# vbronetskyi/nclt-slam-project

Measured on AMD Instinct MI355X. Metric: relocalization frames/sec @640x480, 10k-landmark DB; Hamming-match HBM GB/s, higher is better.
Workload: dtype u8; 1 GPU; 640x480 BGR frames, 10000-record landmark DB (640000 descriptors, rows=fixed64), global relocalization tick per frame: ORB(500) + whole-DB mutual Hamming scan + top-25 PnP-RANSAC(200); frames resident in HBM, every frame's 96-byte result record written to pinned host memory by the tick's last kernel; distinct_frames=32, preroll_steps=20, streams=4, records=10000, descriptors=640000, parallelism=frames sharded across ranks, database replicated, no collective

## Files before the change

### include/reloc.h

```cpp
#ifndef RELOC_H
#define RELOC_H

#include <stdint.h>

#ifdef __cplusplus
extern "C" {
#endif

#define RELOC_OK            0
#define RELOC_E_ARG        (-1)
#define RELOC_E_NODEVICE   (-2)
#define RELOC_E_HIP        (-3)
#define RELOC_E_CAPACITY   (-4)
#define RELOC_E_STATE      (-5)

#define RELOC_ORDER_BGR 0
#define RELOC_ORDER_RGB 1

#define RELOC_OUT_PUBLISHED        0
#define RELOC_OUT_NO_FEATURES      1
#define RELOC_OUT_NO_CANDIDATES    2
#define RELOC_OUT_NO_PNP_ACCEPT    3
#define RELOC_OUT_CONSISTENCY_FAIL 4

// ... 12 lines not shown
    double heading_tol_deg;
    double reproj_max_px;
    double ransac_reproj_px;
    double ransac_confidence;
    double consistency_m;
    double global_reproj_max_px;
    double accum_min_dist_m;
    double accum_depth_min_m;
    double accum_depth_max_m;
    int32_t gray_coeff_bits;
    int32_t reserved0;
} reloc_params;

const char *reloc_last_error(void);
int  reloc_device_count(void);
reloc_ctx *reloc_create(int device, int max_w, int max_h, int max_feat);
void reloc_destroy(reloc_ctx *ctx);
int  reloc_set_stream(reloc_ctx *ctx, void *hip_stream);
int  reloc_sync(reloc_ctx *ctx);
void *reloc_dev_alloc(reloc_ctx *ctx, int64_t bytes);
int  reloc_dev_free(reloc_ctx *ctx, void *p);
int  reloc_h2d(reloc_ctx *ctx, void *dst_dev, const void *src_host, int64_t bytes);
int  reloc_d2d(reloc_ctx *ctx, void *dst_dev, const void *src_dev, int64_t bytes);
void *reloc_host_alloc(int64_t bytes);
int  reloc_host_free(void *p);
void *reloc_get_stream(reloc_ctx *ctx);
int  reloc_d2h(reloc_ctx *ctx, void *dst_host, const void *src_dev, int64_t bytes);
int  reloc_timer_begin(reloc_ctx *ctx);
int  reloc_timer_end(reloc_ctx *ctx, float *ms);
#define RELOC_PROF_DB_SCAN  0
#define RELOC_PROF_MATRIX   1
#define RELOC_PROF_ORB      2
#define RELOC_PROF_PNP      3
#define RELOC_PROF_STEREO   4
#define RELOC_PROF_STEREO_DENSE 5
#define RELOC_PROF_N        6
int  reloc_profile_enable(reloc_ctx *ctx, int on);
int  reloc_profile_get(reloc_ctx *ctx, int which, float *total_ms, int32_t *launches);

int  reloc_get_params(reloc_ctx *ctx, reloc_params *out);
int  reloc_set_params(reloc_ctx *ctx, const reloc_params *p);

int reloc_gray_u8(reloc_ctx *ctx, const uint8_t *img, int w, int h, int stride, int order,
                  uint8_t *gray);
int reloc_orb_detect_compute(reloc_ctx *ctx, const uint8_t *gray, int w, int h, int stride,
                             int nfeatures, float *xy, float *size, float *angle, float *response,
                             int32_t *octave, uint8_t *desc, int32_t *n_out);
int reloc_orb_frame_dev(reloc_ctx *ctx, const uint8_t *img_dev, int w, int h, int stride, int order,
                        int nfeatures);
const uint8_t *reloc_frame_desc_dev(reloc_ctx *ctx);
const float   *reloc_frame_xy_dev(reloc_ctx *ctx);
const int32_t *reloc_frame_count_dev(reloc_ctx *ctx);
int reloc_frame_debug_plane(reloc_ctx *ctx, int what, int level, uint8_t *out, int32_t *w, int32_t *h);

int reloc_set_orb_mask(reloc_ctx *ctx, const uint8_t *mask, int w, int h, int stride);
int reloc_get_orb_mask(reloc_ctx *ctx, int32_t *w, int32_t *h);
int reloc_orb_detect_compute_masked(reloc_ctx *ctx, const uint8_t *gray, int w, int h, int stride, const uint8_t *mask,
                                    int mask_stride, int nfeatures, float *xy, float *size, float *angle,
                                    float *response, int32_t *octave, uint8_t *desc, int32_t *n_out);
int reloc_orb_mask_level(reloc_ctx *ctx, int level, uint8_t *out, int32_t *w, int32_t *h);

int reloc_set_orb_params(reloc_ctx *ctx, int nlevels, double scale_factor, int fast_threshold, int score_type);
int reloc_get_orb_params(reloc_ctx *ctx, int32_t *nlevels, double *scale_factor, int32_t *fast_threshold, int32_t *score_type);
int reloc_orb_detect_compute_params(reloc_ctx *ctx, const uint8_t *gray, int w, int h, int stride, const uint8_t *mask,
                                    int mask_stride, int nfeatures, int nlevels, double scale_factor, int fast_threshold,
                                    int score_type, float *xy, float *size, float *angle, float *response,
                                    int32_t *octave, uint8_t *desc, int32_t *n_out);

int reloc_record_frame(reloc_ctx *ctx, const uint8_t *img, const uint16_t *depth_mm, int w, int h, int order,
                       int nfeatures, float *xy, uint8_t *desc, float *pts3d, int32_t *kp_index,
                       int32_t *n_out, int32_t *n_kp);

int reloc_depth_points(reloc_ctx *ctx, const void *depth, int is_f32, int w, int h, int step, const double K4[4],
                       float zmin, float zmax, float *points, int32_t *n_out);

int reloc_match_mutual(reloc_ctx *ctx, const uint8_t *q, int nq, const uint8_t *t, int nt,
                       int32_t *qidx, int32_t *tidx, int32_t *dist, int32_t *n_out);
int reloc_match_knn2(reloc_ctx *ctx, const uint8_t *q, int nq, const uint8_t *t, int nt,
                     int32_t *idx, int32_t *dist);
int reloc_match_ratio(reloc_ctx *ctx, const uint8_t *q, int nq, const uint8_t *t, int nt, double ratio,
                      int32_t *qidx, int32_t *tidx, int32_t *dist, int32_t *n_out);
#define RELOC_MATCH_CROSS 0
#define RELOC_MATCH_RATIO 1
int reloc_set_match_policy(reloc_ctx *ctx, int policy, double ratio);
int reloc_get_match_policy(reloc_ctx *ctx, int32_t *policy, double *ratio);
int reloc_db_upload(reloc_ctx *ctx, const uint8_t *desc, const float *pts3d, const int64_t *offsets,
                    const double *poses, int64_t n_records);
int64_t reloc_db_records(reloc_ctx *ctx);
int64_t reloc_db_rows(reloc_ctx *ctx);
int reloc_db_reserve(reloc_ctx *ctx, int64_t cap_records, int64_t cap_rows);
int reloc_db_append(reloc_ctx *ctx, const uint8_t *desc, const float *pts3d, const float *kp2d, int n,
                    const double pose[7], const double index_xy[2]);
int reloc_db_select(reloc_ctx *ctx, int slot);
int reloc_db_share(reloc_ctx *dst, reloc_ctx *src);
int reloc_db_fetch(reloc_ctx *ctx, int64_t record, uint8_t *desc, float *pts3d, float *kp2d, double pose[7],
                   double index_xyh[4], int32_t *n);
int reloc_db_match_counts(reloc_ctx *ctx, const uint8_t *cur, int n_cur, int32_t *counts);
int reloc_db_match_counts_dev(reloc_ctx *ctx, const uint8_t *cur_dev, const int32_t *n_cur_dev,
                              int n_cur_max, int32_t *counts_dev);
int reloc_db_ratio_counts(reloc_ctx *ctx, const uint8_t *cur, int n_cur, double ratio, int32_t *counts);
int reloc_hamming_matrix(reloc_ctx *ctx, const uint8_t *a, int64_t na, const uint8_t *b, int64_t nb,
                         uint16_t *out);
int reloc_hamming_matrix_dev(reloc_ctx *ctx, const uint8_t *a_dev, int64_t na, const uint8_t *b_dev,
                             int64_t nb, uint16_t *out_dev);

int reloc_pnp_score(reloc_ctx *ctx, const float *obj, const float *img, int m, const double *Rt, int H,
// ... 154 lines not shown
```

### nclt-slam-project_amd/_native.py

```python
from __future__ import annotations

import ctypes as C
import os

import numpy as np

_HERE = os.path.dirname(os.path.abspath(__file__))
LIB_PATH = (os.environ.get("RELOC_LIB") if os.environ.get("RELOC_DEV") == "1" else None) or os.path.join(_HERE, "csrc", "libreloc_hip.so")

c_ctx = C.c_void_p
i32, i64, u64, f32, f64 = C.c_int32, C.c_int64, C.c_uint64, C.c_float, C.c_double


class RelocError(RuntimeError):
    """Raised for every failure of the native library (the cv2 shim re-raises it as cv2.error)."""


class P:

    @classmethod
    def from_param(cls, a):
        if isinstance(a, np.ndarray):
            if not a.flags.c_contiguous:
                raise RelocError(f"a pointer argument must be a C-contiguous array, got strides {a.strides} for shape {a.shape}")
            return C.c_void_p(a.ctypes.data)
        if isinstance(a, (i32, i64, u64, f32, f64)):
            return C.byref(a)
        return C.c_void_p.from_param(a)


def outs(*types):
    return tuple(t() for t in types)


SIGNATURES = {
    "reloc_last_error": (C.c_char_p, []),
    "reloc_device_count": (C.c_int, []),
    "reloc_create": (c_ctx, [C.c_int, C.c_int, C.c_int, C.c_int]),
    "reloc_destroy": (None, [c_ctx]),
    "reloc_set_stream": (C.c_int, [c_ctx, P]),
    "reloc_sync": (C.c_int, [c_ctx]),
    "reloc_dev_alloc": (C.c_void_p, [c_ctx, i64]),
    "reloc_dev_free": (C.c_int, [c_ctx, P]),
    "reloc_h2d": (C.c_int, [c_ctx, P, P, i64]),
    "reloc_d2h": (C.c_int, [c_ctx, P, P, i64]),
    "reloc_timer_begin": (C.c_int, [c_ctx]),
    "reloc_timer_end": (C.c_int, [c_ctx, P]),
    "reloc_profile_enable": (C.c_int, [c_ctx, C.c_int]),
    "reloc_profile_get": (C.c_int, [c_ctx, C.c_int, P, P]),
    "reloc_gray_u8": (C.c_int, [c_ctx, P, C.c_int, C.c_int, C.c_int, C.c_int, P]),
    "reloc_orb_detect_compute": (C.c_int, [c_ctx, P, C.c_int, C.c_int, C.c_int, C.c_int, P, P, P, P, P, P, P]),
    "reloc_orb_frame_dev": (C.c_int, [c_ctx, P, C.c_int, C.c_int, C.c_int, C.c_int, C.c_int]),
    "reloc_frame_desc_dev": (C.c_void_p, [c_ctx]),
    "reloc_frame_xy_dev": (C.c_void_p, [c_ctx]),
    "reloc_frame_count_dev": (C.c_void_p, [c_ctx]),
    "reloc_frame_debug_plane": (C.c_int, [c_ctx, C.c_int, C.c_int, P, P, P]),
    "reloc_set_orb_mask": (C.c_int, [c_ctx, P, C.c_int, C.c_int, C.c_int]),
    "reloc_get_orb_mask": (C.c_int, [c_ctx, P, P]),
    "reloc_orb_detect_compute_masked": (C.c_int, [c_ctx, P, C.c_int, C.c_int, C.c_int, P, C.c_int, C.c_int, P, P, P, P, P, P, P]),
    "reloc_orb_mask_level": (C.c_int, [c_ctx, C.c_int, P, P, P]),
    "reloc_set_orb_params": (C.c_int, [c_ctx, C.c_int, f64, C.c_int, C.c_int]),
    "reloc_get_orb_params": (C.c_int, [c_ctx, P, P, P, P]),
    "reloc_orb_detect_compute_params": (C.c_int, [c_ctx, P, C.c_int, C.c_int, C.c_int, P, C.c_int, C.c_int, C.c_int, f64, C.c_int,
                                                  C.c_int, P, P, P, P, P, P, P]),
    "reloc_record_frame": (C.c_int, [c_ctx, P, P, C.c_int, C.c_int, C.c_int, C.c_int, P, P, P, P, P, P]),
    "reloc_depth_points": (C.c_int, [c_ctx, P, C.c_int, C.c_int, C.c_int, C.c_int, P, f32, f32, P, P]),
    "reloc_db_ratio_counts": (C.c_int, [c_ctx, P, C.c_int, f64, P]),
    "reloc_match_mutual": (C.c_int, [c_ctx, P, C.c_int, P, C.c_int, P, P, P, P]),
    "reloc_match_knn2": (C.c_int, [c_ctx, P, C.c_int, P, C.c_int, P, P]),
    "reloc_match_ratio": (C.c_int, [c_ctx, P, C.c_int, P, C.c_int, f64, P, P, P, P]),
    "reloc_set_match_policy": (C.c_int, [c_ctx, C.c_int, f64]),
    "reloc_get_match_policy": (C.c_int, [c_ctx, P, P]),
    "reloc_db_upload": (C.c_int, [c_ctx, P, P, P, P, i64]),
    "reloc_db_records": (i64, [c_ctx]),
    "reloc_db_rows": (i64, [c_ctx]),
    "reloc_db_counts_dev": (C.c_void_p, [c_ctx]),
    "reloc_db_match_counts": (C.c_int, [c_ctx, P, C.c_int, P]),
    "reloc_db_match_counts_dev": (C.c_int, [c_ctx, P, P, C.c_int, P]),
    "reloc_hamming_matrix": (C.c_int, [c_ctx, P, i64, P, i64, P]),
    "reloc_hamming_matrix_dev": (C.c_int, [c_ctx, P, i64, P, i64, P]),
    "reloc_pnp_score": (C.c_int, [c_ctx, P, P, C.c_int, P, C.c_int, P, f32, P, P]),
    "reloc_pnp_ransac": (C.c_int, [c_ctx, P, P, C.c_int, P, C.c_int, f32, f64, u64, P, P, P, P, P]),
    "reloc_pnp_debug_hypotheses": (C.c_int, [c_ctx, C.c_int, C.c_int, P, P, P]),
    "reloc_set_camera": (C.c_int, [c_ctx, P, P, P]),
    "reloc_set_distortion": (C.c_int, [c_ctx, P, C.c_int]),
    "reloc_get_distortion": (C.c_int, [c_ctx, P]),
    "reloc_undistort_points": (C.c_int, [c_ctx, P, C.c_int, P, P, P]),
    "reloc_pnp_score_dist": (C.c_int, [c_ctx, P, P, C.c_int, P, C.c_int, P, P, f32, P, P]),
    "reloc_pnp_ransac_dist": (C.c_int, [c_ctx, P, P, C.c_int, P, P, C.c_int, f32, f64, u64, P, P, P, P, P]),
    "reloc_set_clahe": (C.c_int, [c_ctx, f64, C.c_int, C.c_int]),
    "reloc_get_clahe": (C.c_int, [c_ctx, P, P, P]),
    "reloc_clahe_u8": (C.c_int, [c_ctx, P, C.c_int, C.c_int, C.c_int, f64, C.c_int, C.c_int, P]),
    "reloc_set_rectify_map": (C.c_int, [c_ctx, P, P, C.c_int, C.c_int]),
    "reloc_get_rectify_map": (C.c_int, [c_ctx, P, P]),
    "reloc_remap_u8": (C.c_int, [c_ctx, P, C.c_int, C.c_int, C.c_int, C.c_int, P, P, C.c_int, C.c_int, C.c_int, C.c_int, P]),
    "reloc_remap_u16": (C.c_int, [c_ctx, P, C.c_int, C.c_int, C.c_int, P, C.c_int, C.c_int, C.c_int, P]),
    "reloc_convert_maps": (C.c_int, [c_ctx, P, P, C.c_int, C.c_int, C.c_int, P, P]),
    "reloc_resize_u8": (C.c_int, [c_ctx, P, C.c_int, C.c_int, C.c_int, C.c_int, P, C.c_int, C.c_int, f64, f64, C.c_int]),
    "reloc_resize_u16": (C.c_int, [c_ctx, P, C.c_int, C.c_int, C.c_int, P, C.c_int, C.c_int, f64, f64]),
    "reloc_set_resize": (C.c_int, [c_ctx, C.c_int, C.c_int, C.c_int, C.c_int]),
    "reloc_get_resize": (C.c_int, [c_ctx, P, P, P, P]),
    "reloc_bayer_u8": (C.c_int, [c_ctx, P, C.c_int, C.c_int, C.c_int, C.c_int, P]),
    "reloc_set_bayer": (C.c_int, [c_ctx, C.c_int]),
    "reloc_get_bayer": (C.c_int, [c_ctx, P]),
    "reloc_cvt_gray_u8": (C.c_int, [c_ctx, P, C.c_int, C.c_int, C.c_int, C.c_int, P]),
    "reloc_yuv422_bgr_u8": (C.c_int, [c_ctx, P, C.c_int, C.c_int, C.c_int, C.c_int, C.c_int, P]),
    "reloc_set_pixel_format": (C.c_int, [c_ctx, C.c_int]),
    "reloc_get_pixel_format": (C.c_int, [c_ctx, P]),
    "reloc_set_stereo": (C.c_int, [c_ctx, f64, C.c_int, C.c_int, C.c_int, C.c_int]),
# ... 167 lines not shown
```

### nclt-slam-project_amd/csrc/reloc_orb.hip

```cpp
#include <math.h>

#include "../../include/reloc_orb_pattern.h"
#include "reloc_internal.h"
#include "reloc_pixels.h"

static_assert(HARRIS_CHUNK == 1024, "k_harris reads one dword per thread");

__constant__ signed char c_pattern[RELOC_ORB_NTESTS * 4];
__constant__ int c_umax[16] = {15, 15, 15, 15, 14, 14, 14, 13, 13, 12, 11, 10, 9, 8, 6, 3};
__constant__ signed char c_ring_dx[16] = {0, 1, 2, 3, 3, 3, 2, 1, 0, -1, -2, -3, -3, -3, -2, -1};
__constant__ signed char c_ring_dy[16] = {3, 3, 2, 1, 0, -1, -2, -3, -3, -3, -2, -1, 0, 1, 2, 3};

__device__ __forceinline__ int find_level(const int *base, int id)
{
    int l = 0;
#pragma unroll
    for (int k = 1; k < NLEV; ++k) l += id >= base[k];
    return l;
}


struct OrbBatch { OrbFrame f[RELOC_BATCH_MAX]; };

__device__ __forceinline__ void pyr_tab_index(const OrbTable *__restrict__ tab, const PyrTile &T, const int (&tbase)[NLEV + 1], int i,
// ... 308 lines not shown
        constexpr u32 sel_o = (u32)(o + 1) | 0x0C00u | (u32)(o + 3) << 16 | 0x0C000000u;
        const u32 ve = __builtin_amdgcn_perm(w[DY + 3][q + 1], w[DY + 3][q], sel_e);
        const u32 vo = __builtin_amdgcn_perm(w[DY + 3][q + 1], w[DY + 3][q], sel_o);
        tb[0] = ve + nb[0]; tb[1] = vo + nb[1];
        td[0] = nd[0] - ve; td[1] = nd[1] - vo;
    }
    template <int K>
    __device__ __forceinline__ void ring(u32 (&tb)[2], u32 (&td)[2]) const
    {
        constexpr int dx[16] = {0, 1, 2, 3, 3, 3, 2, 1, 0, -1, -2, -3, -3, -3, -2, -1};
        constexpr int dy[16] = {3, 3, 2, 1, 0, -1, -2, -3, -3, -3, -2, -1, 0, 1, 2, 3};
        flags<dx[K], dy[K]>(tb, td);
    }
    __device__ __forceinline__ bool candidate() const
    {
        u32 b0[2], d0[2], b4[2], d4[2], b8[2], d8[2], b12[2], d12[2];
        ring<0>(b0, d0); ring<4>(b4, d4); ring<8>(b8, d8); ring<12>(b12, d12);
        u32 any = 0;
#pragma unroll
        for (int j = 0; j < 2; ++j) {
            any |= (b0[j] & b4[j]) | (b8[j] & b12[j]) | ((b0[j] | b4[j]) & (b8[j] | b12[j]));
            any |= (d0[j] & d4[j]) | (d8[j] & d12[j]) | ((d0[j] | d4[j]) & (d8[j] | d12[j]));
        }
        return (any & 0x80008000u) != 0;
    }
    template <int K>
    __device__ __forceinline__ void shift_in(u32 (&mb)[2], u32 (&md)[2]) const
    {
        u32 tb[2], td[2];
        ring<K>(tb, td);
#pragma unroll
        for (int j = 0; j < 2; ++j) {
            mb[j] = (tb[j] & 0x80008000u) | ((mb[j] >> 1) & 0x7FFF7FFFu);
            md[j] = (td[j] & 0x80008000u) | ((md[j] >> 1) & 0x7FFF7FFFu);
        }
        if constexpr (K < 15) shift_in<K + 1>(mb, md);
    }
    __device__ __forceinline__ void masks(u32 (&mb)[2], u32 (&md)[2]) const
    {
        mb[0] = mb[1] = md[0] = md[1] = 0;
        shift_in<0>(mb, md);
    }
};

constexpr int FT_P = FT / 4 + 3;
static_assert(FT == 32, "fast_nms_tile maps 256 lanes to 32 rows x 8 dwords");
template <bool MASKED, int THR>
__device__ __forceinline__ void fast_nms_tile(const OrbTable *__restrict__ tab, const uint8_t *__restrict__ pyr,
                                              uint8_t *__restrict__ nms, int32_t *__restrict__ hist, int bid,
                                              const uint8_t *__restrict__ mask)
{
    __shared__ u32 s_img4[(FT + 8) * FT_P];
    __shared__ u32 s_sc4[(FT + 2) * (FT + 4) / 4];
    __shared__ unsigned short s_corner[(FT + 2) * (FT + 2)];
    __shared__ int s_nc;
    __shared__ int s_hist[256];
    const uint8_t *const s_img = reinterpret_cast<const uint8_t *>(s_img4);
    uint8_t *const s_sc = reinterpret_cast<uint8_t *>(s_sc4);
    const int l = find_level(tab->fast_tile_base, bid);
    const OrbLevel L = tab->lev[l];
    const int tile = bid - tab->fast_tile_base[l];
    const int tx = L.stride / FT;
    const int x0 = (tile % tx) * FT, y0 = (tile / tx) * FT;
    const int tid = threadIdx.x;
    const int e = RELOC_ORB_EDGE;
    const int thr = THR ? THR : tab->fast_thr;
    uint8_t *out = nms + L.off;
    const bool live = L.quota > 0 && x0 + FT > e && x0 < L.w - e && y0 + FT > e && y0 < L.h - e;
    if (!live) {
        const int y = y0 + tid / 8, x = x0 + (tid % 8) * 4;
        if (y < L.h) *reinterpret_cast<u32 *>(out + (size_t)y * L.stride + x) = 0;
        return;
    }
    s_hist[tid] = 0;
    const uint8_t *src = pyr + L.off;
    const int IS = 4 * FT_P;
    {
        const int r16 = tid >> 4, c16 = tid & 15;
        u32 v[3];
#pragma unroll
        for (int t = 0; t < 3; ++t) {
            const int ry = 16 * t + r16;
            if (c16 < FT / 4 + 2 && ry < FT + 8) {
                const int gy = min(max(y0 + ry - 4, 0), L.h - 1);
                v[t] = halo_dword<false>(src + (size_t)gy * L.stride, x0 - 4 + 4 * c16, L.w);
            }
        }
#pragma unroll
        for (int t = 0; t < 3; ++t) {
            const int ry = 16 * t + r16;
            if (c16 < FT / 4 + 2 && ry < FT + 8) s_img4[ry * FT_P + c16] = v[t];
        }
    }
    for (int i = tid; i < (FT + 2) * (FT + 4) / 4; i += 256) s_sc4[i] = 0;
    if (tid == 0) s_nc = 0;
    __syncthreads();
    const int SS = FT + 4;
    {
        const int ry = 1 + (tid >> 3), g = tid & 7, rx = 1 + 4 * g;
        u32 w[7][3];
#pragma unroll
        for (int r = 0; r < 7; ++r)
#pragma unroll
            for (int q = 0; q < 3; ++q) w[r][q] = s_img4[(ry + r) * FT_P + g + q];
        const FastQuad Q(w, thr);
        if (__any(Q.candidate())) {
            u32 mb[2], md[2];
            Q.masks(mb, md);
            const int gy = y0 + ry - 1;
            const bool row_in = gy >= 3 && gy < L.h - 3;
#pragma unroll
            for (int k = 0; k < 4; ++k) {
                const u32 sel = (k & 2) ? 0x03020302u : 0x01000100u;
                const bool br = fast_run9(__builtin_amdgcn_perm(mb[k & 1], mb[k & 1], sel));
                const bool dk = fast_run9(__builtin_amdgcn_perm(md[k & 1], md[k & 1], sel));
                const int gx = x0 + rx - 1 + k;
                if ((br || dk) && row_in && gx >= 3 && gx < L.w - 3)
                    s_corner[atomicAdd(&s_nc, 1)] = (unsigned short)((ry << 6) | (rx + k) | (br ? 0 : 0x8000));
            }
        }
    }
    {
        const int i = tid;
        const int ry = i < FT + 2 ? 0 : (i < 2 * (FT + 2) ? FT + 1 : (i < 3 * FT + 4 ? i - (2 * FT + 3) : i - (3 * FT + 3)));
        const int rx = i < FT + 2 ? i : (i < 2 * (FT + 2) ? i - (FT + 2) : (i < 3 * FT + 4 ? 0 : FT + 1));
        const int gy = y0 + ry - 1, gx = x0 + rx - 1;
        int pol = 0;
        bool cand = false;
        const uint8_t *pc = s_img + (ry + 3) * IS + (rx + 3);
        const bool inside = i < 4 * FT + 4 && gx >= 3 && gx < L.w - 3 && gy >= 3 && gy < L.h - 3;
        if (inside) {
            const int c = pc[0];
            const int v0 = (int)pc[3 * IS] - c, v4 = (int)pc[3] - c, v8 = (int)pc[-3 * IS] - c, v12 = (int)pc[-3] - c;
            const int nb = (v0 > thr) + (v4 > thr) + (v8 > thr) + (v12 > thr);
            const int nd = (v0 < -thr) + (v4 < -thr) + (v8 < -thr) + (v12 < -thr);
            cand = nb >= 2 || nd >= 2;
        }
        if (tid < 3 * 64 && __any(cand)) {
            if (cand) pol = fast_is_corner(pc, IS, thr);
        }
        if (pol) s_corner[atomicAdd(&s_nc, 1)] = (unsigned short)((ry << 6) | rx | (pol < 0 ? 0x8000 : 0));
    }
    __syncthreads();
    for (int i = tid; i < s_nc; i += 256) {
        const int e16 = s_corner[i], ry = (e16 >> 6) & 63, rx = e16 & 63;
        s_sc[ry * SS + rx] = (uint8_t)fast_corner_score(s_img + (ry + 3) * IS + (rx + 3), IS, thr, (e16 & 0x8000) ? -1 : 1);
    }
    __syncthreads();
    {
        const int ry = tid / 8, rx4 = (tid % 8) * 4;
        u32 word = 0;
        u32 keep = 0;
        if constexpr (MASKED)
            if (y0 + ry < L.h) keep = *reinterpret_cast<const u32 *>(mask + L.off + (size_t)(y0 + ry) * L.stride + x0 + rx4);
#pragma unroll
        for (int k = 0; k < 4; ++k) {
            const int gx = x0 + rx4 + k, gy = y0 + ry;
            const uint8_t *s = s_sc + (ry + 1) * SS + (rx4 + k + 1);
            const int c = (!MASKED || ((keep >> (8 * k)) & 0xFF)) ? s[0] : 0;
            if (c && gx >= e && gx < L.w - e && gy >= e && gy < L.h - e && c > s[-1] && c > s[1] && c > s[-SS - 1] &&
                c > s[-SS] && c > s[-SS + 1] && c > s[SS - 1] && c > s[SS] && c > s[SS + 1]) {
                word |= (u32)c << (8 * k);
                atomicAdd(&s_hist[c], 1);
            }
        }
        const int gy = y0 + ry;
        if (gy < L.h) *reinterpret_cast<u32 *>(out + (size_t)gy * L.stride + x0 + rx4) = word;
    }
    __syncthreads();
    if (s_hist[tid]) atomicAdd(&hist[l * 256 + tid], s_hist[tid]);
}

template <bool MASKED, int THR>
__global__ __launch_bounds__(256) void k_fast_blur(const OrbTable *__restrict__ tab, const uint8_t *__restrict__ pyr,
                                                   uint8_t *__restrict__ nms, int32_t *__restrict__ hist,
                                                   uint8_t *__restrict__ blur, int n_fast, const uint8_t *__restrict__ mask)
{
    RELOC_SMALL_KERNEL_PRIO();
    if ((int)blockIdx.x < n_fast) fast_nms_tile<MASKED, THR>(tab, pyr, nms, hist, (int)blockIdx.x, mask);
    else blur7_tile(tab, pyr, blur, (int)blockIdx.x - n_fast);
}
template <bool MASKED, int THR>
__global__ __launch_bounds__(256) void k_fast_blur_batch(OrbBatch b, int n_fast)
{
    RELOC_SMALL_KERNEL_PRIO();
    const OrbFrame &F = b.f[blockIdx.y];
    if ((int)blockIdx.x < n_fast) fast_nms_tile<MASKED, THR>(F.tab, F.pyr, F.nms, F.hist, (int)blockIdx.x, F.mask);
    else blur7_tile(F.tab, F.pyr, F.blur, (int)blockIdx.x - n_fast);
}

__global__ __launch_bounds__(256) void k_mask_level(const OrbTable *__restrict__ tab, const int32_t *__restrict__ rz,
                                                    uint8_t *__restrict__ mp, int l)
{
    const OrbLevel S = tab->lev[l - 1], D = tab->lev[l];
    const int x4 = 4 * (int)(blockIdx.x * 256 + threadIdx.x), y = (int)blockIdx.y;
    if (x4 >= D.stride || y >= D.h) return;
    const int32_t *xo = rz + tab->rz_off[l][0], *xc = rz + tab->rz_off[l][1];
    const int sy0 = rz[tab->rz_off[l][2] + y], sy1 = sy0 + 1 < S.h ? sy0 + 1 : S.h - 1;
    const u32 b = (u32)rz[tab->rz_off[l][3] + y], one = 1u << RELOC_RESIZE_COEF_BITS;
    const uint8_t *r0 = mp + S.off + (size_t)sy0 * S.stride, *r1 = mp + S.off + (size_t)sy1 * S.stride;
    u32 out = 0;
#pragma unroll
    for (int k = 0; k < 4; ++k) {
        if (x4 + k < D.w) {
            const int k0 = xo[x4 + k], k1 = k0 + 1 < S.w ? k0 + 1 : S.w - 1;
            const u32 a = (u32)xc[x4 + k];
            const u32 h0 = (u32)r0[k0] * (one - a) + (u32)r0[k1] * a;
            const u32 h1 = (u32)r1[k0] * (one - a) + (u32)r1[k1] * a;
            const u32 v = (h0 * (one - b) + h1 * b + (1u << 15)) >> 16;
            if (v > RELOC_ORB_MASK_THRESH) out |= v << (8 * k);
        }
    }
    *reinterpret_cast<u32 *>(mp + D.off + (size_t)y * D.stride + x4) = out;
}

__device__ int stage1_cut_wave(const int32_t *__restrict__ hist_l, int n_keep, int lane, int thr)
{
    const int4 h = *reinterpret_cast<const int4 *>(hist_l + 4 * lane);
    const int mine = h.x + h.y + h.z + h.w;
    int incl = mine;
#pragma unroll
    for (int d = 1; d < 64; d <<= 1) {
        const int v = __shfl_down(incl, d);
        if (lane + d < 64) incl += v;
    }
    const int above = incl - mine;
    const int c3 = h.w + above, c2 = h.z + c3, c1 = h.y + c2, c0 = h.x + c1;
    const int total = __builtin_amdgcn_readlane(c0, 0);
    int cut0 = thr;
    if (total > n_keep) {
        const int s = c3 >= n_keep ? 3 : (c2 >= n_keep ? 2 : (c1 >= n_keep ? 1 : (c0 >= n_keep ? 0 : -1)));
        cut0 = (int)wave_max_u32(s < 0 ? 0u : (unsigned)(4 * lane + s + 1)) - 1;
    }
    unsigned best = 0;
    const int cs[4] = {c0, c1, c2, c3};
#pragma unroll
    for (int k = 3; k >= 0; --k) {
        const int s = 4 * lane + k;
        if (s >= cut0 && (cs[k] <= RELOC_ORB_STAGE1_CAP || s == 255)) best = (unsigned)(256 - s);
    }
    return 256 - (int)wave_max_u32(best);
}

__device__ __forceinline__ void harris_terms(const uint8_t *p, int step, int lane, int &a, int &b, int &c)
{
    a = b = c = 0;
    if (lane < 49) {
        const int dy = lane / 7 - 3, dx = lane % 7 - 3;
        const uint8_t *q = p + dy * step + dx;
        const int ix = (q[1] - q[-1]) * 2 + (q[-step + 1] - q[-step - 1]) + (q[step + 1] - q[step - 1]);
        const int iy = (q[step] - q[-step]) * 2 + (q[step - 1] - q[-step - 1]) + (q[step + 1] - q[-step + 1]);
        a = ix * ix; b = iy * iy; c = ix * iy;
    }
}

__device__ __forceinline__ float harris_finish(int a, int b, int c)
{
    a = wave_sum_i32(a);
    b = wave_sum_i32(b);
    c = wave_sum_i32(c);
    const float scale = __fdiv_rn(1.f, (float)((1 << 2) * RELOC_HARRIS_BLOCK) * 255.f);
    const float s2 = __fmul_rn(scale, scale), s3 = __fmul_rn(s2, scale), s4 = __fmul_rn(s3, scale);
    const float fa = (float)a, fb = (float)b, fc = (float)c;
    const float t1 = __fmul_rn(fa, fb), t2 = __fmul_rn(fc, fc), t3 = __fadd_rn(fa, fb);
    const float t4 = __fmul_rn(RELOC_HARRIS_K, t3), t5 = __fmul_rn(t4, t3);
    const float t6 = __fsub_rn(t1, t2), t7 = __fsub_rn(t6, t5);
    return __fmul_rn(t7, s4);
}

enum { ORB_MODE_DEFAULT = 0, ORB_MODE_HARRIS = 1, ORB_MODE_FAST = 2 };
template <int MODE>
__device__ __forceinline__ void harris_body(const OrbTable *__restrict__ tab, const uint8_t *__restrict__ pyr,
                                                const uint8_t *__restrict__ nms, const int32_t *__restrict__ hist,
                                                int32_t *__restrict__ cand_cnt, u32 *__restrict__ cand_key,
                                                float *__restrict__ cand_resp, int32_t *__restrict__ dbg_cut)
{
    __shared__ int s_cut;
    __shared__ int s_n, s_base;
    __shared__ u32 s_list[HARRIS_CHUNK];
    const int thr = MODE == ORB_MODE_DEFAULT ? RELOC_FAST_THRESHOLD : tab->fast_thr;
    const int l = find_level(tab->flat_base, blockIdx.x);
    const OrbLevel L = tab->lev[l];
    if (L.quota <= 0 || L.w <= 2 * RELOC_ORB_EDGE || L.h <= 2 * RELOC_ORB_EDGE) return;
    const int64_t idx0 = ((int64_t)(blockIdx.x - tab->flat_base[l]) * 256 + threadIdx.x) * (HARRIS_CHUNK / 256);
    const int64_t total = (int64_t)L.stride * L.h;
    u32 v = 0;
    if (idx0 < total) v = *reinterpret_cast<const u32 *>(nms + L.off + idx0);
    const bool any = v != 0;
    if (threadIdx.x == 0) s_n = 0;
    if (!__syncthreads_or(any)) return;
    if (threadIdx.x < 64) {
        const int c = stage1_cut_wave(hist + l * 256, MODE == ORB_MODE_FAST ? L.quota : 2 * L.quota, threadIdx.x, thr);
        if (threadIdx.x == 0) {
            s_cut = c;
            if (dbg_cut) dbg_cut[l] = c;
        }
    }
    __syncthreads();
    const int cut = s_cut;
    if constexpr (MODE == ORB_MODE_FAST) {
        if (any) {
#pragma unroll
            for (int k = 0; k < HARRIS_CHUNK / 256; ++k) {
                const int sc = (v >> (8 * k)) & 0xFF;
                if (sc && sc >= cut) {
                    const int64_t idx = idx0 + k;
                    const int y = (int)(idx / L.stride), x = (int)(idx % L.stride);
                    const int pos = atomicAdd(&cand_cnt[l], 1);
                    if (pos < RELOC_ORB_STAGE1_CAP) {
                        cand_key[(size_t)l * RELOC_ORB_STAGE1_CAP + pos] = ((u32)y << 16) | (u32)x;
                        cand_resp[(size_t)l * RELOC_ORB_STAGE1_CAP + pos] = (float)sc;
                    }
                }
            }
        }
        return;
    }
    if (any) {
#pragma unroll
        for (int k = 0; k < HARRIS_CHUNK / 256; ++k) {
            const int sc = (v >> (8 * k)) & 0xFF;
            if (sc && sc >= cut) {
                const int64_t idx = idx0 + k;
                const int y = (int)(idx / L.stride), x = (int)(idx % L.stride);
                s_list[atomicAdd(&s_n, 1)] = ((u32)y << 16) | (u32)x;
            }
        }
    }
    __syncthreads();
    const int n = s_n;
    const int lane = threadIdx.x & 63, wave = threadIdx.x >> 6;
    const uint8_t *img = pyr + L.off;
    int base_ret = 0;
    if (threadIdx.x == 0 && n > 0) base_ret = atomicAdd(&cand_cnt[l], n);
    auto terms = [&](u32 key, int &a, int &b, int &c) {
        harris_terms(img + (size_t)(key >> 16) * L.stride + (key & 0xFFFF), L.stride, lane, a, b, c);
    };
    int i = wave * 2;
    const bool first = i < n;
    u32 k0 = 0, k1 = 0;
    int a0 = 0, b0 = 0, c0 = 0, a1 = 0, b1 = 0, c1 = 0;
    float h0 = 0.f, h1 = 0.f;
    if (first) {
        k0 = s_list[i]; k1 = s_list[i + 1 < n ? i + 1 : i];
        terms(k0, a0, b0, c0);
        terms(k1, a1, b1, c1);
    }
    if (threadIdx.x == 0) s_base = base_ret;
    if (first) { h0 = harris_finish(a0, b0, c0); h1 = harris_finish(a1, b1, c1); }
    __syncthreads();
    const int base = s_base;
    auto put = [&](int at, u32 key, float r) {
        const int pos = base + at;
        if (pos < RELOC_ORB_STAGE1_CAP) {
            cand_key[(size_t)l * RELOC_ORB_STAGE1_CAP + pos] = key;
            cand_resp[(size_t)l * RELOC_ORB_STAGE1_CAP + pos] = r;
        }
    };
    if (first && lane == 0) {
        put(i, k0, h0);
        if (i + 1 < n) put(i + 1, k1, h1);
    }
    for (i += 8; i < n; i += 8) {
        k0 = s_list[i]; k1 = s_list[i + 1 < n ? i + 1 : i];
        terms(k0, a0, b0, c0);
        terms(k1, a1, b1, c1);
        h0 = harris_finish(a0, b0, c0);
        h1 = harris_finish(a1, b1, c1);
        if (lane == 0) {
            put(i, k0, h0);
            if (i + 1 < n) put(i + 1, k1, h1);
        }
    }
}
template <int MODE>
__global__ __launch_bounds__(256) void k_harris(const OrbTable *__restrict__ tab, const uint8_t *__restrict__ pyr,
                                                const uint8_t *__restrict__ nms, const int32_t *__restrict__ hist,
                                                int32_t *__restrict__ cand_cnt, u32 *__restrict__ cand_key,
                                                float *__restrict__ cand_resp, int32_t *__restrict__ dbg_cut)
{
    RELOC_SMALL_KERNEL_PRIO();
    harris_body<MODE>(tab, pyr, nms, hist, cand_cnt, cand_key, cand_resp, dbg_cut);
}
template <int MODE>
__global__ __launch_bounds__(256) void k_harris_batch(OrbBatch b)
{
    RELOC_SMALL_KERNEL_PRIO();
    const OrbFrame &F = b.f[blockIdx.y];
    harris_body<MODE>(F.tab, F.pyr, F.nms, F.hist, F.cand_cnt, F.cand_key, F.cand_resp, F.dbg_cut);
}

__device__ __forceinline__ void select_body(const OrbTable *__restrict__ tab, const int32_t *__restrict__ cand_cnt,
                                                 const u32 *__restrict__ cand_key, const float *__restrict__ cand_resp,
                                                 int32_t *__restrict__ kp_cnt, u32 *__restrict__ kp_key,
                                                 float *__restrict__ kp_resp)
{
    __shared__ u32 s_key[RELOC_ORB_STAGE1_CAP];
    __shared__ float s_resp[RELOC_ORB_STAGE1_CAP];
    __shared__ u32 s_kidx[RELOC_ORB_STAGE1_CAP];
    __shared__ int s_nk;
    const int l = blockIdx.x;
    const int quota = tab->lev[l].quota;
    const int M = min(cand_cnt[l], RELOC_ORB_STAGE1_CAP);
    const int tid = threadIdx.x;
    if (tid == 0) s_nk = 0;
    for (int i = tid; i < M; i += 1024) {
        s_key[i] = cand_key[(size_t)l * RELOC_ORB_STAGE1_CAP + i];
        s_resp[i] = cand_resp[(size_t)l * RELOC_ORB_STAGE1_CAP + i];
    }
    __syncthreads();
    for (int i = tid; i < M; i += 1024) {
        const float r = s_resp[i];
        int greater = 0;
        for (int j = 0; j < M; ++j) greater += s_resp[j] > r;
        if (greater < quota) s_kidx[atomicAdd(&s_nk, 1)] = (u32)i;
    }
    __syncthreads();
    const int K = s_nk;
    for (int i = tid; i < K; i += 1024) {
        const u32 src = s_kidx[i];
        const u32 key = s_key[src];
        int pos = 0;
        for (int j = 0; j < K; ++j) pos += s_key[s_kidx[j]] < key;
        kp_key[(size_t)l * RELOC_ORB_STAGE1_CAP + pos] = key;
        kp_resp[(size_t)l * RELOC_ORB_STAGE1_CAP + pos] = s_resp[src];
// ... 465 lines not shown
    OrbMaskStage &m = ctx->orb.mask;
    if (!mask || (w == 0 && h == 0)) {
        m.w = m.h = 0;
        m.built = false;
        return RELOC_OK;
    }
    ARG_CHECK(w >= 1 && h >= 1 && stride >= w, "reloc_set_orb_mask: the size is not positive or the stride is below the width");
    if (w > ctx->max_w || h > ctx->max_h) { reloc_set_error("detection mask exceeds ctx capacity"); return RELOC_E_CAPACITY; }
    if (int rc = mask_alloc(ctx)) return rc;
    HIP_TRY(hipStreamSynchronize(ctx->stream));
    m.w = m.h = 0;
    m.built = false;
    if (m.last == m.pyr) m.last = nullptr;
    if (int rc = mask_upload(ctx, m.pyr, mask, w, h, stride)) return rc;
    HIP_TRY(hipStreamSynchronize(ctx->stream));
    m.w = w; m.h = h;
    return RELOC_OK;
}

RELOC_API int reloc_get_orb_mask(reloc_ctx *ctx, int32_t *w, int32_t *h)
{
    ARG_CHECK_CTX(ctx, w && h, "reloc_get_orb_mask");
    *w = ctx->orb.mask.w; *h = ctx->orb.mask.h;
    return RELOC_OK;
}

RELOC_API int reloc_orb_mask_level(reloc_ctx *ctx, int level, uint8_t *out, int32_t *w, int32_t *h)
{
    ARG_CHECK_CTX(ctx, out && w && h && level >= 0 && level < NLEV, "reloc_orb_mask_level");
    const OrbMaskStage &m = ctx->orb.mask;
    if (!m.last || m.last_w != ctx->orb.w || m.last_h != ctx->orb.h) { reloc_set_error("no masked frame processed yet"); return RELOC_E_STATE; }
    const OrbLevel &L = ctx->orb.tab.lev[level];
    if (L.w < 1 || L.h < 1) { *w = *h = 0; return RELOC_OK; }
    HIP_TRY(hipMemcpy2DAsync(out, L.w, m.last + L.off, L.stride, L.w, L.h, hipMemcpyDeviceToHost, ctx->stream));
    HIP_TRY(hipStreamSynchronize(ctx->stream));
    *w = L.w;
    *h = L.h;
    return RELOC_OK;
}

RELOC_API int reloc_frame_debug_plane(reloc_ctx *ctx, int what, int level, uint8_t *out, int32_t *w, int32_t *h)
{
    ARG_CHECK_CTX(ctx, out && w && h && what >= 0 && what <= 2 && level >= 0 && level < NLEV, "reloc_frame_debug_plane");
    if (!ctx->orb.w) { reloc_set_error("no frame processed yet"); return RELOC_E_STATE; }
    const OrbLevel &L = ctx->orb.tab.lev[level];
    if (L.w < 1 || L.h < 1) { *w = *h = 0; return RELOC_OK; }
    const uint8_t *src = (what == 0 ? ctx->orb.buf.pyr : what == 1 ? ctx->orb.buf.blur : ctx->orb.buf.nms) + L.off;
    HIP_TRY(hipMemcpy2DAsync(out, L.w, src, L.stride, L.w, L.h, hipMemcpyDeviceToHost, ctx->stream));
    HIP_TRY(hipStreamSynchronize(ctx->stream));
    *w = L.w;
    *h = L.h;
    return RELOC_OK;
}
```

### nclt-slam-project_amd/engine.py

```python
from __future__ import annotations

import ctypes as C

import numpy as np

from . import _native as N
from ._native import f32, f64, i32
from .front_end import PIXEL_FORMATS, frame_shape_ok, pixel_format_setting

K4_DEFAULT = np.array([320.0, 320.0, 320.0, 240.0], dtype=np.float64)

OUTCOME_NAMES = {0: "published", 1: "curr_no_features", 2: "no_candidates", 3: "no_pnp_accept",
                 4: "consistency_fail"}

MATCH_POLICIES = {"cross": 0, "ratio": 1}
MATCH_POLICY_RULE = "policy must be RELOC_MATCH_CROSS (0) or RELOC_MATCH_RATIO (1)"
MATCH_RATIO_RULE = "ratio must be finite and in (0, 1]"


def match_policy_setting(policy, ratio):
    name = policy.lower() if isinstance(policy, str) else {v: k for k, v in MATCH_POLICIES.items()}.get(policy)
    if name not in MATCH_POLICIES:
        raise ValueError(f'match_policy {policy!r}: {MATCH_POLICY_RULE}, "cross" or "ratio"')
    try:
# ... 529 lines not shown
            raise N.RelocError("stereo_frame_points: step must be an integer >= 1")
        step = int(step)
        pts = np.empty((-(-w // step) * -(-h // step), 3), np.float32)
        n = i32()
        self._api.reloc_stereo_frame_points(self._ctx, right_engine._ctx, frame, right_frame, w, h, int(order_rgb), step,
                                            float(zmin), float(zmax), pts, n)
        return pts[: n.value].copy()

    def stereo_dense_debug(self):
        px = self.max_w * self.max_h
        mm = np.zeros(px, np.uint16); disp = np.zeros(px, np.float32); st = np.zeros(px, np.uint8)
        w, h = N.outs(i32, i32)
        self._api.reloc_stereo_dense_debug(self._ctx, mm, disp, st, w, h)
        k, shape = w.value * h.value, (h.value, w.value)
        return mm[:k].reshape(shape).copy(), disp[:k].reshape(shape).copy(), st[:k].reshape(shape).copy()

    def filter_speckles(self, img: np.ndarray, new_val: int, max_speckle_size: int, max_diff: int) -> np.ndarray:
        if not isinstance(img, np.ndarray) or img.dtype != np.int16 or img.ndim != 2 or img.size == 0 or not img.flags.writeable:
            raise N.RelocError("filter_speckles: expected a writable, non-empty (H, W) int16 array")
        for name, v in (("new_val", new_val), ("max_speckle_size", max_speckle_size), ("max_diff", max_diff)):
            if int(v) != v:
                raise N.RelocError(f"filter_speckles: {name} must be an integer")
        if not -32768 <= int(new_val) <= 32767:
            raise N.RelocError("filter_speckles: new_val must fit int16")
        if int(max_speckle_size) < 0 or int(max_diff) < 0:
            raise N.RelocError("filter_speckles: max_speckle_size and max_diff must be >= 0")
        h, w = img.shape
        limit, diff = min(int(max_speckle_size), 2 ** 31 - 1), min(int(max_diff), 65536)
        if img.strides[1] == 2 and img.strides[0] % 2 == 0 and (h == 1 or img.strides[0] >= 2 * w):
            self._api.reloc_filter_speckles(self._ctx, img.ctypes.data, w, h, w if h == 1 else img.strides[0] // 2, int(new_val), limit, diff)
        else:
            dense = np.ascontiguousarray(img)
            self._api.reloc_filter_speckles(self._ctx, dense, w, h, w, int(new_val), limit, diff)
            img[...] = dense
        return img

    def set_stereo_speckle(self, window: int = 0, range: int = 1):
        for name, v in (("window", window), ("range", range)):
            if int(v) != v:
                raise N.RelocError(f"set_stereo_speckle: {name} must be an integer")
        self._api.reloc_set_stereo_speckle(self._ctx, int(window), int(range))

    def get_stereo_speckle(self):
        win, rng = N.outs(i32, i32)
        self._api.reloc_get_stereo_speckle(self._ctx, win, rng)
        return win.value, rng.value

    def frame_debug_plane(self, what: int, level: int) -> np.ndarray:
        buf = np.empty(self.max_w * self.max_h, np.uint8)
        w, h = N.outs(i32, i32)
        self._api.reloc_frame_debug_plane(self._ctx, what, level, buf, w, h)
        return buf[: w.value * h.value].reshape(h.value, w.value).copy()

    @staticmethod
    def _desc(a, name):
        a = np.asarray(a)
        if a.dtype != np.uint8 or a.ndim != 2 or a.shape[1] != 32:
            raise N.RelocError(f"{name}: descriptors must be (N, 32) uint8, got {a.dtype} {a.shape}")
        return np.ascontiguousarray(a)

    def match_mutual(self, q, t):
        q = self._desc(q, "match"); t = self._desc(t, "match")
        cap = max(min(len(q), len(t)), 1)
        qi = np.empty(cap, np.int32); ti = np.empty(cap, np.int32); dd = np.empty(cap, np.int32)
        n = i32()
        self._api.reloc_match_mutual(self._ctx, q, len(q), t, len(t), qi, ti, dd, n)
        return qi[: n.value].copy(), ti[: n.value].copy(), dd[: n.value].copy()

    def match_knn2(self, q, t):
        q = self._desc(q, "knnMatch"); t = self._desc(t, "knnMatch")
        idx = np.empty((len(q), 2), np.int32); dist = np.empty((len(q), 2), np.int32)
        self._api.reloc_match_knn2(self._ctx, q, len(q), t, len(t), idx, dist)
        return idx, dist

    def match_ratio(self, q, t, ratio: float = 0.8):
        q = self._desc(q, "match_ratio"); t = self._desc(t, "match_ratio")
        cap = max(len(q), 1)
        qi = np.empty(cap, np.int32); ti = np.empty(cap, np.int32); dd = np.empty(cap, np.int32)
        n = i32()
        self._api.reloc_match_ratio(self._ctx, q, len(q), t, len(t), float(ratio), qi, ti, dd, n)
        return qi[: n.value].copy(), ti[: n.value].copy(), dd[: n.value].copy()

    def db_upload(self, desc, pts3d, offsets, poses):
        desc = self._desc(desc, "db_upload") if len(desc) else np.zeros((0, 32), np.uint8)
        pts3d = np.ascontiguousarray(pts3d, np.float32).reshape(-1, 3)
        offsets = np.ascontiguousarray(offsets, np.int64)
        poses = np.ascontiguousarray(poses, np.float64).reshape(-1, 7)
        if len(offsets) != len(poses) + 1 or offsets[-1] != len(desc) or len(pts3d) != len(desc):
            raise N.RelocError("db_upload: inconsistent array sizes")
        self._api.reloc_db_upload(self._ctx, desc, pts3d, offsets, poses, len(poses))

    def db_reserve(self, cap_records: int, cap_rows: int):
        self._api.reloc_db_reserve(self._ctx, int(cap_records), int(cap_rows))

    def db_append(self, desc, pts3d, pose, keypoints_2d=None, index_xy=None):
        desc = self._desc(desc, "db_append") if len(desc) else np.zeros((0, 32), np.uint8)
        pts3d = np.ascontiguousarray(pts3d, np.float32).reshape(-1, 3)
        if len(pts3d) != len(desc):
            raise N.RelocError("db_append: descriptor / point counts differ")
        kp = None if keypoints_2d is None else np.ascontiguousarray(keypoints_2d, np.float32).reshape(-1, 2)
        if kp is not None and len(kp) != len(desc):
            raise N.RelocError("db_append: descriptor / keypoint counts differ")
        pose = np.ascontiguousarray(pose, np.float64).reshape(7)
        ixy = None if index_xy is None else np.ascontiguousarray(index_xy, np.float64).reshape(2)
        self._api.reloc_db_append(self._ctx, desc, pts3d, kp, len(desc), pose, ixy)

# ... 481 lines not shown
```

Measured before the change: 7644 frames/s.

## Sparsify FAST border pass and pack Harris response into quarter-wave DPP reductions

The FAST tile kernel no longer runs a dense per-thread border-ring test. It now rescans only the 3x3 neighbours of interior corners that touch the tile edge, then does NMS over the corner list into a shared output tile, with an early exit that writes zeros when a tile has no corners. The Harris stage1 kernel evaluates four candidates per wavefront, 16 lanes each, and reduces with DPP row operations instead of whole-wave reductions. A debug API for dumping stage-1 histograms and candidates is also added. The intent is to cut wasted lanes and reduction latency in ORB detection, at the cost of extra atomics, shared memory, and a possible change in corner ordering.

```diff
diff --git a/include/reloc.h b/include/reloc.h
--- a/include/reloc.h
+++ b/include/reloc.h
@@ -88,6 +88,8 @@
 const float   *reloc_frame_xy_dev(reloc_ctx *ctx);
 const int32_t *reloc_frame_count_dev(reloc_ctx *ctx);
 int reloc_frame_debug_plane(reloc_ctx *ctx, int what, int level, uint8_t *out, int32_t *w, int32_t *h);
+int reloc_orb_debug_stage1(reloc_ctx *ctx, int32_t *hist, int32_t *cut, int32_t *cand_cnt, uint32_t *cand_key,
+                           float *cand_resp);
 
 int reloc_set_orb_mask(reloc_ctx *ctx, const uint8_t *mask, int w, int h, int stride);
 int reloc_get_orb_mask(reloc_ctx *ctx, int32_t *w, int32_t *h);
diff --git a/nclt-slam-project_amd/_native.py b/nclt-slam-project_amd/_native.py
--- a/nclt-slam-project_amd/_native.py
+++ b/nclt-slam-project_amd/_native.py
@@ -55,6 +55,7 @@
     "reloc_frame_xy_dev": (C.c_void_p, [c_ctx]),
     "reloc_frame_count_dev": (C.c_void_p, [c_ctx]),
     "reloc_frame_debug_plane": (C.c_int, [c_ctx, C.c_int, C.c_int, P, P, P]),
+    "reloc_orb_debug_stage1": (C.c_int, [c_ctx, P, P, P, P, P]),
     "reloc_set_orb_mask": (C.c_int, [c_ctx, P, C.c_int, C.c_int, C.c_int]),
     "reloc_get_orb_mask": (C.c_int, [c_ctx, P, P]),
     "reloc_orb_detect_compute_masked": (C.c_int, [c_ctx, P, C.c_int, C.c_int, C.c_int, P, C.c_int, C.c_int, P, P, P, P, P, P, P]),
diff --git a/nclt-slam-project_amd/csrc/reloc_orb.hip b/nclt-slam-project_amd/csrc/reloc_orb.hip
--- a/nclt-slam-project_amd/csrc/reloc_orb.hip
+++ b/nclt-slam-project_amd/csrc/reloc_orb.hip
@@ -384,11 +384,13 @@
 {
     __shared__ u32 s_img4[(FT + 8) * FT_P];
     __shared__ u32 s_sc4[(FT + 2) * (FT + 4) / 4];
+    __shared__ u32 s_out4[FT * FT / 4];
     __shared__ unsigned short s_corner[(FT + 2) * (FT + 2)];
-    __shared__ int s_nc;
+    __shared__ int s_nc, s_nr;
     __shared__ int s_hist[256];
     const uint8_t *const s_img = reinterpret_cast<const uint8_t *>(s_img4);
     uint8_t *const s_sc = reinterpret_cast<uint8_t *>(s_sc4);
+    uint8_t *const s_out = reinterpret_cast<uint8_t *>(s_out4);
     const int l = find_level(tab->fast_tile_base, bid);
     const OrbLevel L = tab->lev[l];
     const int tile = bid - tab->fast_tile_base[l];
@@ -405,6 +407,7 @@
         return;
     }
     s_hist[tid] = 0;
+    s_out4[tid] = 0;
     const uint8_t *src = pyr + L.off;
     const int IS = 4 * FT_P;
     {
@@ -425,7 +428,7 @@
         }
     }
     for (int i = tid; i < (FT + 2) * (FT + 4) / 4; i += 256) s_sc4[i] = 0;
-    if (tid == 0) s_nc = 0;
+    if (tid == 0) s_nc = s_nr = 0;
     __syncthreads();
     const int SS = FT + 4;
     {
@@ -452,54 +455,54 @@
             }
         }
     }
-    {
-        const int i = tid;
-        const int ry = i < FT + 2 ? 0 : (i < 2 * (FT + 2) ? FT + 1 : (i < 3 * FT + 4 ? i - (2 * FT + 3) : i - (3 * FT + 3)));
-        const int rx = i < FT + 2 ? i : (i < 2 * (FT + 2) ? i - (FT + 2) : (i < 3 * FT + 4 ? 0 : FT + 1));
-        const int gy = y0 + ry - 1, gx = x0 + rx - 1;
-        int pol = 0;
-        bool cand = false;
+    __syncthreads();
+    const int nc1 = s_nc;
+    const int oy = y0 + tid / 8, ox = x0 + (tid % 8) * 4;
+    if (nc1 == 0) {
+        if (oy < L.h) *reinterpret_cast<u32 *>(out + (size_t)oy * L.stride + ox) = 0;
+        return;
+    }
+    for (int i = tid; i < nc1; i += 256) {
+        const int e16 = s_corner[i], ry = (e16 >> 6) & 63, rx = e16 & 63;
+        if (ry == 1 || ry == FT || rx == 1 || rx == FT) {
+#pragma unroll
+            for (int d = 0; d < 9; ++d) {
+                const int ny = ry + d / 3 - 1, nx = rx + d % 3 - 1;
+                const int gy = y0 + ny - 1, gx = x0 + nx - 1;
+                if ((ny == 0 || ny == FT + 1 || nx == 0 || nx == FT + 1) && gx >= 3 && gx < L.w - 3 && gy >= 3 && gy < L.h - 3) {
+                    const u32 bit = 0xFFu << (8 * (nx & 3));
+                    if (!(atomicOr(&s_sc4[(ny * SS + nx) >> 2], bit) & bit))
+                        s_corner[nc1 + atomicAdd(&s_nr, 1)] = (unsigned short)((ny << 6) | nx);
+                }
+            }
+        }
+    }
+    __syncthreads();
+    for (int i = tid; i < nc1 + s_nr; i += 256) {
+        const int e16 = s_corner[i], ry = (e16 >> 6) & 63, rx = e16 & 63;
         const uint8_t *pc = s_img + (ry + 3) * IS + (rx + 3);
-        const bool inside = i < 4 * FT + 4 && gx >= 3 && gx < L.w - 3 && gy >= 3 && gy < L.h - 3;
-        if (inside) {
-            const int c = pc[0];
-            const int v0 = (int)pc[3 * IS] - c, v4 = (int)pc[3] - c, v8 = (int)pc[-3 * IS] - c, v12 = (int)pc[-3] - c;
-            const int nb = (v0 > thr) + (v4 > thr) + (v8 > thr) + (v12 > thr);
-            const int nd = (v0 < -thr) + (v4 < -thr) + (v8 < -thr) + (v12 < -thr);
-            cand = nb >= 2 || nd >= 2;
-        }
-        if (tid < 3 * 64 && __any(cand)) {
-            if (cand) pol = fast_is_corner(pc, IS, thr);
-        }
-        if (pol) s_corner[atomicAdd(&s_nc, 1)] = (unsigned short)((ry << 6) | rx | (pol < 0 ? 0x8000 : 0));
+        int pol = (e16 & 0x8000) ? -1 : 1;
+        if (i >= nc1) pol = fast_is_corner(pc, IS, thr);
+        int sc = 0;
+        if (pol) sc = fast_corner_score(pc, IS, thr, pol);
+        s_sc[ry * SS + rx] = (uint8_t)sc;
     }
     __syncthreads();
-    for (int i = tid; i < s_nc; i += 256) {
+    for (int i = tid; i < nc1; i += 256) {
         const int e16 = s_corner[i], ry = (e16 >> 6) & 63, rx = e16 & 63;
-        s_sc[ry * SS + rx] = (uint8_t)fast_corner_score(s_img + (ry + 3) * IS + (rx + 3), IS, thr, (e16 & 0x8000) ? -1 : 1);
+        const int gx = x0 + rx - 1, gy = y0 + ry - 1;
+        const uint8_t *s = s_sc + ry * SS + rx;
+        int c = s[0];
+        if constexpr (MASKED)
+            if (!mask[L.off + (size_t)gy * L.stride + gx]) c = 0;
+        if (c && gx >= e && gx < L.w - e && gy >= e && gy < L.h - e && c > s[-1] && c > s[1] && c > s[-SS - 1] &&
+            c > s[-SS] && c > s[-SS + 1] && c > s[SS - 1] && c > s[SS] && c > s[SS + 1]) {
+            s_out[(ry - 1) * FT + (rx - 1)] = (uint8_t)c;
+            atomicAdd(&s_hist[c], 1);
+        }
     }
     __syncthreads();
-    {
-        const int ry = tid / 8, rx4 = (tid % 8) * 4;
-        u32 word = 0;
-        u32 keep = 0;
-        if constexpr (MASKED)
-            if (y0 + ry < L.h) keep = *reinterpret_cast<const u32 *>(mask + L.off + (size_t)(y0 + ry) * L.stride + x0 + rx4);
-#pragma unroll
-        for (int k = 0; k < 4; ++k) {
-            const int gx = x0 + rx4 + k, gy = y0 + ry;
-            const uint8_t *s = s_sc + (ry + 1) * SS + (rx4 + k + 1);
-            const int c = (!MASKED || ((keep >> (8 * k)) & 0xFF)) ? s[0] : 0;
-            if (c && gx >= e && gx < L.w - e && gy >= e && gy < L.h - e && c > s[-1] && c > s[1] && c > s[-SS - 1] &&
-                c > s[-SS] && c > s[-SS + 1] && c > s[SS - 1] && c > s[SS] && c > s[SS + 1]) {
-                word |= (u32)c << (8 * k);
-                atomicAdd(&s_hist[c], 1);
-            }
-        }
-        const int gy = y0 + ry;
-        if (gy < L.h) *reinterpret_cast<u32 *>(out + (size_t)gy * L.stride + x0 + rx4) = word;
-    }
-    __syncthreads();
+    if (oy < L.h) *reinterpret_cast<u32 *>(out + (size_t)oy * L.stride + ox) = s_out4[tid];
     if (s_hist[tid]) atomicAdd(&hist[l * 256 + tid], s_hist[tid]);
 }
 
@@ -574,23 +577,28 @@
     return 256 - (int)wave_max_u32(best);
 }
 
-__device__ __forceinline__ void harris_terms(const uint8_t *p, int step, int lane, int &a, int &b, int &c)
-{
-    a = b = c = 0;
-    if (lane < 49) {
-        const int dy = lane / 7 - 3, dx = lane % 7 - 3;
-        const uint8_t *q = p + dy * step + dx;
-        const int ix = (q[1] - q[-1]) * 2 + (q[-step + 1] - q[-step - 1]) + (q[step + 1] - q[step - 1]);
-        const int iy = (q[step] - q[-step]) * 2 + (q[step - 1] - q[-step - 1]) + (q[step + 1] - q[-step + 1]);
-        a = ix * ix; b = iy * iy; c = ix * iy;
-    }
-}
-
-__device__ __forceinline__ float harris_finish(int a, int b, int c)
-{
-    a = wave_sum_i32(a);
-    b = wave_sum_i32(b);
-    c = wave_sum_i32(c);
+__device__ __forceinline__ float harris_quarter(const uint8_t *p, int step, int j)
+{
+    const int r = j < 14 ? j >> 1 : 6, half = j & 1;
+    const uint8_t *q = p + (r - 3) * step + 4 * half - 3;
+    int u[6], m[6], d[6];
+#pragma unroll
+    for (int k = 0; k < 6; ++k) { u[k] = q[-step + k - 1]; m[k] = q[k - 1]; d[k] = q[step + k - 1]; }
+    int a = 0, b = 0, c = 0;
+#pragma unroll
+    for (int k = 0; k < 4; ++k) {
+        const int ix = (m[k + 2] - m[k]) * 2 + (u[k + 2] - u[k]) + (d[k + 2] - d[k]);
+        const int iy = (d[k + 1] - u[k + 1]) * 2 + (d[k] - u[k]) + (d[k + 2] - u[k + 2]);
+        const bool on = j < 14 && (k < 3 || !half);
+        a += on ? ix * ix : 0; b += on ? iy * iy : 0; c += on ? ix * iy : 0;
+    }
+#define RELOC_DPP_STEP(x, ctrl) x += __builtin_amdgcn_update_dpp(0, x, ctrl, 0xF, 0xF, false);
+#define RELOC_ROW_SUM(x) RELOC_DPP_STEP(x, 0xB1) RELOC_DPP_STEP(x, 0x4E) RELOC_DPP_STEP(x, 0x141) RELOC_DPP_STEP(x, 0x140)
+    RELOC_ROW_SUM(a)
+    RELOC_ROW_SUM(b)
+    RELOC_ROW_SUM(c)
+#undef RELOC_ROW_SUM
+#undef RELOC_DPP_STEP
     const float scale = __fdiv_rn(1.f, (float)((1 << 2) * RELOC_HARRIS_BLOCK) * 255.f);
     const float s2 = __fmul_rn(scale, scale), s3 = __fmul_rn(s2, scale), s4 = __fmul_rn(s3, scale);
     const float fa = (float)a, fb = (float)b, fc = (float)c;
@@ -665,44 +673,30 @@
     const uint8_t *img = pyr + L.off;
     int base_ret = 0;
     if (threadIdx.x == 0 && n > 0) base_ret = atomicAdd(&cand_cnt[l], n);
-    auto terms = [&](u32 key, int &a, int &b, int &c) {
-        harris_terms(img + (size_t)(key >> 16) * L.stride + (key & 0xFFFF), L.stride, lane, a, b, c);
+    const int sub = lane >> 4, j = lane & 15;
+    auto response = [&](int at, u32 &key) {
+        key = s_list[at < n ? at : n - 1];
+        return harris_quarter(img + (size_t)(key >> 16) * L.stride + (key & 0xFFFF), L.stride, j);
     };
-    int i = wave * 2;
-    const bool first = i < n;
-    u32 k0 = 0, k1 = 0;
-    int a0 = 0, b0 = 0, c0 = 0, a1 = 0, b1 = 0, c1 = 0;
-    float h0 = 0.f, h1 = 0.f;
-    if (first) {
-        k0 = s_list[i]; k1 = s_list[i + 1 < n ? i + 1 : i];
-        terms(k0, a0, b0, c0);
-        terms(k1, a1, b1, c1);
-    }
+    int t = wave * 4;
+    const bool first = t < n;
+    u32 key = 0;
+    float r = 0.f;
+    if (first) r = response(t + sub, key);
     if (threadIdx.x == 0) s_base = base_ret;
-    if (first) { h0 = harris_finish(a0, b0, c0); h1 = harris_finish(a1, b1, c1); }
     __syncthreads();
     const int base = s_base;
-    auto put = [&](int at, u32 key, float r) {
+    auto put = [&](int at) {
         const int pos = base + at;
-        if (pos < RELOC_ORB_STAGE1_CAP) {
+        if (j == 0 && at < n && pos < RELOC_ORB_STAGE1_CAP) {
             cand_key[(size_t)l * RELOC_ORB_STAGE1_CAP + pos] = key;
             cand_resp[(size_t)l * RELOC_ORB_STAGE1_CAP + pos] = r;
         }
     };
-    if (first && lane == 0) {
-        put(i, k0, h0);
-        if (i + 1 < n) put(i + 1, k1, h1);
-    }
-    for (i += 8; i < n; i += 8) {
-        k0 = s_list[i]; k1 = s_list[i + 1 < n ? i + 1 : i];
-        terms(k0, a0, b0, c0);
-        terms(k1, a1, b1, c1);
-        h0 = harris_finish(a0, b0, c0);
-        h1 = harris_finish(a1, b1, c1);
-        if (lane == 0) {
-            put(i, k0, h0);
-            if (i + 1 < n) put(i + 1, k1, h1);
-        }
+    if (first) put(t + sub);
+    for (t += 16; t < n; t += 16) {
+        r = response(t + sub, key);
+        put(t + sub);
     }
 }
 template <int MODE>
@@ -1274,3 +1268,19 @@
     *h = L.h;
     return RELOC_OK;
 }
+
+RELOC_API int reloc_orb_debug_stage1(reloc_ctx *ctx, int32_t *hist, int32_t *cut, int32_t *cand_cnt, uint32_t *cand_key,
+                                     float *cand_resp)
+{
+    ARG_CHECK_CTX(ctx, hist && cut && cand_cnt && cand_key && cand_resp, "reloc_orb_debug_stage1");
+    if (!ctx->orb.w) { reloc_set_error("no frame processed yet"); return RELOC_E_STATE; }
+    const OrbFrame &b = ctx->orb.buf;
+    const size_t s1 = (size_t)NLEV * RELOC_ORB_STAGE1_CAP;
+    HIP_TRY(hipMemcpyAsync(hist, b.hist, NLEV * 256 * sizeof(int32_t), hipMemcpyDeviceToHost, ctx->stream));
+    HIP_TRY(hipMemcpyAsync(cut, b.dbg_cut, NLEV * sizeof(int32_t), hipMemcpyDeviceToHost, ctx->stream));
+    HIP_TRY(hipMemcpyAsync(cand_cnt, b.cand_cnt, NLEV * sizeof(int32_t), hipMemcpyDeviceToHost, ctx->stream));
+    HIP_TRY(hipMemcpyAsync(cand_key, b.cand_key, s1 * sizeof(uint32_t), hipMemcpyDeviceToHost, ctx->stream));
+    HIP_TRY(hipMemcpyAsync(cand_resp, b.cand_resp, s1 * sizeof(float), hipMemcpyDeviceToHost, ctx->stream));
+    HIP_TRY(hipStreamSynchronize(ctx->stream));
+    return RELOC_OK;
+}
diff --git a/nclt-slam-project_amd/engine.py b/nclt-slam-project_amd/engine.py
--- a/nclt-slam-project_amd/engine.py
+++ b/nclt-slam-project_amd/engine.py
@@ -605,6 +605,14 @@
         self._api.reloc_frame_debug_plane(self._ctx, what, level, buf, w, h)
         return buf[: w.value * h.value].reshape(h.value, w.value).copy()
 
+    def orb_debug_stage1(self):
+        cap = 4096
+        hist = np.empty((8, 256), np.int32); cut = np.empty(8, np.int32); cnt = np.empty(8, np.int32)
+        key = np.empty((8, cap), np.uint32); resp = np.empty((8, cap), np.float32)
+        self._api.reloc_orb_debug_stage1(self._ctx, hist, cut, cnt, key, resp)
+        n = np.minimum(cnt, cap)
+        return dict(hist=hist, cut=cut, cand_cnt=cnt, cand=[(key[l, :n[l]].copy(), resp[l, :n[l]].copy()) for l in range(8)])
+
     @staticmethod
     def _desc(a, name):
         a = np.asarray(a)
```

After: 7673 frames/s (median of 6 runs). No clear change (+0.4%).
